# Aceinna/gnss-ins-sim

Measured on AMD Instinct MI355X. Metric: Monte-Carlo IMU samples integrated/sec, higher is better.
Workload: dtype f64

## Files before the change

### gnss-ins-sim_amd/csrc/ginsim_api.hip

```cpp
#include <hip/hip_runtime.h>
#include <chrono>

#include <cmath>
#include <cstdarg>
#include <cstdio>
#include <cstring>
#include <string>
#include <vector>

#include "ginsim.h"
#include "ginsim_oallan.h"
#include "allan.hpp"
#include "oallan.hpp"
#include "comm.hpp"
#include "launch.hpp"
#include "placed.hpp"

namespace ginsim {

static thread_local std::string g_err;

void set_error(const char* fmt, ...) {
    char buf[512];
    va_list ap;
    va_start(ap, fmt);
    vsnprintf(buf, sizeof(buf), fmt, ap);
    va_end(ap);
    g_err = buf;
}

}

using namespace ginsim;

struct ginsim_ctx {
    int device;
    hipStream_t stream;
    hipEvent_t ev0, ev1;
    std::vector<hipEvent_t> pool;
    void* ws[4] = {nullptr, nullptr, nullptr, nullptr};
    size_t ws_bytes[4] = {0, 0, 0, 0};
    double* allan_host = nullptr;
    size_t allan_host_doubles = 0;
    int max_grid_y = 65535;
    ginsim::Comm* comm = nullptr;
    double* comm_recv = nullptr;
    ginsim_stats* comm_host = nullptr;
    hipEvent_t comm_ev[8] = {};
    bool comm_pending[8] = {};
    ginsim_stats* stat_slots = nullptr;
    hipEvent_t stat_ev[8] = {};
    bool stat_pending[8] = {};
    unsigned long long* selftest = nullptr;
};

static hipError_t scratch(ginsim_ctx* c, int slot, size_t bytes, void** out) {
    if (c->ws_bytes[slot] < bytes) {
        if (c->ws[slot]) {
            hipError_t e = hipStreamSynchronize(c->stream);
            if (e != hipSuccess) return e;
            e = hipFree(c->ws[slot]);
            if (e != hipSuccess) return e;
            c->ws[slot] = nullptr;
            c->ws_bytes[slot] = 0;
        }
        const size_t want = bytes + bytes / 4 + 4096;
        hipError_t e = hipMalloc(&c->ws[slot], want);
        if (e != hipSuccess) return e;
        c->ws_bytes[slot] = want;
    }
    *out = c->ws[slot];
    return hipSuccess;
}

#define HIP_TRY(expr)                                                                         \
    do {                                                                                      \
        hipError_t e_ = (expr);                                                               \
        if (e_ != hipSuccess) {                                                               \
            set_error("%s failed: %s (%s:%d)", #expr, hipGetErrorString(e_), __FILE__, __LINE__); \
            if (e_ == hipErrorOutOfMemory) { (void)hipGetLastError(); return GINSIM_ERR_NOMEM; } \
            return GINSIM_ERR_HIP;                                                            \
        }                                                                                     \
    } while (0)

#define REQUIRE(cond, ...)            \
    do {                              \
        if (!(cond)) {                \
            set_error(__VA_ARGS__);   \
            return GINSIM_ERR_ARG;    \
        }                             \
    } while (0)

struct DevBuf {
    void* p = nullptr;
    ~DevBuf() { if (p) (void)hipFree(p); }
    hipError_t alloc(size_t bytes) { return hipMalloc(&p, bytes ? bytes : 8); }
    template <class T> T* as() const { return reinterpret_cast<T*>(p); }
};

template <class Launch>
static int gather_run(const char* who, ginsim_ctx* c, const void* series, int32_t ncomp, int64_t n, int64_t runs, const int64_t* run_ids,
                      int32_t nsel, double* host_out, Launch launch) {
    REQUIRE(c && series && run_ids && host_out, "%s: NULL argument", who);
    REQUIRE(ncomp >= 1 && n >= 1 && runs >= 1 && nsel >= 1, "%s: bad sizes", who);
    for (int i = 0; i < nsel; ++i)
        REQUIRE(run_ids[i] >= 0 && run_ids[i] < runs, "%s: run id %lld out of range", who, (long long)run_ids[i]);
    HIP_TRY(hipSetDevice(c->device));
    DevBuf ids, out;
    const size_t out_bytes = sizeof(double) * (size_t)nsel * n * ncomp;
    HIP_TRY(ids.alloc(sizeof(int64_t) * nsel));
    HIP_TRY(out.alloc(out_bytes));
    HIP_TRY(hipMemcpyAsync(ids.p, run_ids, sizeof(int64_t) * nsel, hipMemcpyHostToDevice, c->stream));
    HIP_TRY(launch(ids.as<int64_t>(), out.as<double>()));
    HIP_TRY(hipMemcpyAsync(host_out, out.p, out_bytes, hipMemcpyDeviceToHost, c->stream));
    HIP_TRY(hipStreamSynchronize(c->stream));
    return GINSIM_OK;
}

template <class Launch>
static int traj_run(ginsim_ctx* c, TrajView v, size_t body, double* host_out, size_t out_bytes, Launch launch) {
    HIP_TRY(hipSetDevice(c->device));
    void* ws = nullptr;
    HIP_TRY(scratch(c, 2, body + sizeof(int64_t) * (size_t)v.m, &ws));
    if (v.samples) {
        int64_t* d_samples = reinterpret_cast<int64_t*>(reinterpret_cast<char*>(ws) + body);
        HIP_TRY(hipMemcpyAsync(d_samples, v.samples, sizeof(int64_t) * (size_t)v.m, hipMemcpyHostToDevice, c->stream));
        v.samples = d_samples;
    }
    HIP_TRY(launch(v, ws));
    if (out_bytes) HIP_TRY(hipMemcpyAsync(host_out, ws, out_bytes, hipMemcpyDeviceToHost, c->stream));
    HIP_TRY(hipStreamSynchronize(c->stream));
    return GINSIM_OK;
}
// ... 125 lines not shown
    int64_t mmax = 0;
    allan_factors(n, fs, mult, &mmax);
    if (mult.empty()) return GINSIM_OK;
    REQUIRE((int)mult.size() <= kOallanMaxFactors && n < ((int64_t)1 << 31), "oallan: series too long");
    const char* e = getenv("GINSIM_OALLAN_TILE");
    const bool tiles = !(e && e[0] == '0' && e[1] == 0);
    const int64_t C = oallan_tile_payload(), H = oallan_tile_halo(), W = oallan_stream_item();
    F.count = (int32_t)mult.size();
    int64_t records = 0;
    for (int i = 0; i < F.count; ++i) {
        const int64_t m = mult[i], terms = n - 2 * m + 1;
        const bool tile = tiles && 2 * m <= H && i == P.tile && P.tile < kOallanTileFactors;
        if (tile) ++P.tile;
        const int64_t per = tile ? C : W;
        F.m[i] = (int32_t)m;
        F.nparts[i] = (int32_t)((terms + per - 1) / per);
        F.offset[i] = (int32_t)records;
        records += F.nparts[i];
    }
    F.records = (int32_t)records;
    const auto pad = [](size_t b) { return (b + 255) & ~(size_t)255; };
    P.b_records = pad(sizeof(double) * (size_t)records * (size_t)nseries);
    if (F.count > P.tile) {
        P.theta_stride = (n + 2) & ~(int64_t)1;
        P.b_theta = pad(sizeof(double) * (size_t)P.theta_stride * (size_t)nseries);
        P.b_sums = pad(sizeof(double) * (size_t)(n / oallan_scan_chunk() + 1) * (size_t)nseries);
    }
    return GINSIM_OK;
}

extern "C" {

int ginsim_abi_version(void) { return GINSIM_ABI_VERSION; }

const char* ginsim_last_error(void) { return g_err.c_str(); }

int ginsim_device_count(int* count) {
    REQUIRE(count, "device_count: NULL output");
    int n = 0;
    const hipError_t e = hipGetDeviceCount(&n);
    if (e != hipSuccess) {
        *count = 0;
        set_error("hipGetDeviceCount: %s", hipGetErrorString(e));
        return GINSIM_ERR_NODEV;
    }
    *count = n;
    return GINSIM_OK;
}

int ginsim_create(int device, ginsim_ctx** out) {
    REQUIRE(out, "create: NULL output");
    *out = nullptr;
    int n = 0;
    if (hipGetDeviceCount(&n) != hipSuccess || n < 1) {
        set_error("no HIP device visible (the engine has no CPU fallback)");
        return GINSIM_ERR_NODEV;
    }
    REQUIRE(device >= 0 && device < n, "create: device %d out of range [0,%d)", device, n);
    HIP_TRY(hipSetDevice(device));
    ginsim_ctx* c = new ginsim_ctx();
    c->device = device;
    HIP_TRY(hipStreamCreateWithFlags(&c->stream, hipStreamNonBlocking));
    HIP_TRY(hipEventCreate(&c->ev0));
    HIP_TRY(hipEventCreate(&c->ev1));
    HIP_TRY(hipDeviceGetAttribute(&c->max_grid_y, hipDeviceAttributeMaxGridDimY, device));
    ginsim::placed_context_created(device);
    *out = c;
    return GINSIM_OK;
}

int ginsim_destroy(ginsim_ctx* c) {
    if (!c) return GINSIM_OK;
    (void)hipSetDevice(c->device);
    (void)hipStreamSynchronize(c->stream);
    (void)hipEventDestroy(c->ev0);
    (void)hipEventDestroy(c->ev1);
    for (hipEvent_t e : c->pool)
        if (e) (void)hipEventDestroy(e);
    for (void* w : c->ws)
        if (w) (void)hipFree(w);
    for (hipEvent_t e : c->stat_ev)
        if (e) (void)hipEventDestroy(e);
    if (c->stat_slots) (void)hipHostFree(c->stat_slots);
    if (c->allan_host) (void)hipHostFree(c->allan_host);
    if (c->selftest) (void)hipFree(c->selftest);
    if (c->comm) ginsim::comm_destroy(c->comm);
    if (c->comm_recv) (void)hipFree(c->comm_recv);
    if (c->comm_host) (void)hipHostFree(c->comm_host);
    for (hipEvent_t e : c->comm_ev)
        if (e) (void)hipEventDestroy(e);
    ginsim::vib_psd_drop_plans(c->stream);
    (void)hipStreamDestroy(c->stream);
    ginsim::placed_free_owner(c->device, c);
    ginsim::placed_context_destroyed(c->device);
    delete c;
    return GINSIM_OK;
}

int ginsim_device_name(ginsim_ctx* c, char* buf, size_t cap) {
    REQUIRE(c && buf && cap > 0, "device_name: bad arguments");
    hipDeviceProp_t prop;
    HIP_TRY(hipGetDeviceProperties(&prop, c->device));
    snprintf(buf, cap, "%s (%s, %d CUs)", prop.name, prop.gcnArchName, prop.multiProcessorCount);
    return GINSIM_OK;
}

int ginsim_malloc(ginsim_ctx* c, size_t bytes, void** dptr) {
    REQUIRE(c && dptr, "malloc: bad arguments");
    HIP_TRY(hipSetDevice(c->device));
    HIP_TRY(hipMalloc(dptr, bytes ? bytes : 8));
    return GINSIM_OK;
}

int ginsim_placed_configure(ginsim_ctx* c, const ginsim_placed_options* o) {
    REQUIRE(c && o, "placed_configure: bad arguments");
    return ginsim::placed_configure(c->device, *o);
}

int ginsim_placed_reserve(ginsim_ctx* c, size_t bytes) {
    REQUIRE(c, "placed_reserve: NULL context");
    return ginsim::placed_reserve(c->device, c->stream, bytes);
}

int ginsim_malloc_placed(ginsim_ctx* c, size_t bytes, void** dptr) {
    REQUIRE(c && dptr, "malloc_placed: bad arguments");
    return ginsim::placed_malloc(c->device, c->stream, bytes, c, dptr);
}

int ginsim_placed_release(ginsim_ctx* c) {
    REQUIRE(c, "placed_release: NULL context");
    HIP_TRY(hipSetDevice(c->device));
    HIP_TRY(hipStreamSynchronize(c->stream));
    return ginsim::placed_release(c->device, false);
}

int ginsim_placed_info_get(ginsim_ctx* c, ginsim_placed_info* out) {
    REQUIRE(c && out, "placed_info_get: bad arguments");
    ginsim::placed_info(c->device, out);
    return GINSIM_OK;
}

int ginsim_mem_info(ginsim_ctx* c, size_t* free_bytes, size_t* total_bytes) {
    REQUIRE(c && free_bytes && total_bytes, "mem_info: bad arguments");
    HIP_TRY(hipSetDevice(c->device));
    HIP_TRY(hipMemGetInfo(free_bytes, total_bytes));
    return GINSIM_OK;
}

int ginsim_host_alloc(ginsim_ctx* c, size_t bytes, void** hptr) {
    REQUIRE(c && hptr, "host_alloc: bad arguments");
    HIP_TRY(hipSetDevice(c->device));
    HIP_TRY(hipHostMalloc(hptr, bytes ? bytes : 8, hipHostMallocDefault));
    return GINSIM_OK;
}

int ginsim_host_free(ginsim_ctx* c, void* hptr) {
    if (!hptr) return GINSIM_OK;
    if (c) {
        HIP_TRY(hipSetDevice(c->device));
        HIP_TRY(hipStreamSynchronize(c->stream));
    }
    HIP_TRY(hipHostFree(hptr));
    return GINSIM_OK;
}

int ginsim_free(ginsim_ctx* c, void* dptr) {
// ... 442 lines not shown
int ginsim_loose_kernel_name(const ginsim_mc_params* mc, const ginsim_loose_params* p, char* buf, size_t cap) {
    REQUIRE(buf && cap > 0, "loose_kernel_name: bad arguments");
    return loose_entry(LOOSE_PLAIN, nullptr, LooseLaunch{mc, p, nullptr, nullptr, nullptr, nullptr, buf, cap});
}

int ginsim_loose_run(ginsim_ctx* c, const ginsim_mc_params* mc, const ginsim_loose_params* p) {
    REQUIRE(c, "loose_run: NULL argument");
    return loose_entry(LOOSE_PLAIN, c, LooseLaunch{mc, p});
}

int ginsim_loose_cons_kernel_name(const ginsim_mc_params* mc, const ginsim_loose_params* p, const ginsim_loose_cons_params* cons,
                                  char* buf, size_t cap) {
    REQUIRE(buf && cap > 0, "loose_cons_kernel_name: bad arguments");
    return loose_entry(LOOSE_CONS, nullptr, LooseLaunch{mc, p, cons, nullptr, nullptr, nullptr, buf, cap});
}

int ginsim_loose_cons_run(ginsim_ctx* c, const ginsim_mc_params* mc, const ginsim_loose_params* p, const ginsim_loose_cons_params* cons) {
    REQUIRE(c, "loose_cons_run: NULL argument");
    return loose_entry(LOOSE_CONS, c, LooseLaunch{mc, p, cons});
}

int ginsim_loose_mag_kernel_name(const ginsim_mc_params* mc, const ginsim_loose_params* p, const ginsim_loose_mag_params* mag,
                                 char* buf, size_t cap) {
    REQUIRE(buf && cap > 0, "loose_mag_kernel_name: bad arguments");
    return loose_entry(LOOSE_MAG, nullptr, LooseLaunch{mc, p, nullptr, mag, nullptr, nullptr, buf, cap});
}

int ginsim_loose_mag_run(ginsim_ctx* c, const ginsim_mc_params* mc, const ginsim_loose_params* p, const ginsim_loose_mag_params* mag) {
    REQUIRE(c, "loose_mag_run: NULL argument");
    return loose_entry(LOOSE_MAG, c, LooseLaunch{mc, p, nullptr, mag});
}

int ginsim_loose_scale_kernel_name(const ginsim_mc_params* mc, const ginsim_loose_params* p, const ginsim_loose_scale_params* scale,
                                   char* buf, size_t cap) {
    REQUIRE(buf && cap > 0, "loose_scale_kernel_name: bad arguments");
    return loose_entry(LOOSE_SCALE, nullptr, LooseLaunch{mc, p, nullptr, nullptr, scale, nullptr, buf, cap});
}

int ginsim_loose_scale_run(ginsim_ctx* c, const ginsim_mc_params* mc, const ginsim_loose_params* p, const ginsim_loose_scale_params* scale) {
    REQUIRE(c, "loose_scale_run: NULL argument");
    return loose_entry(LOOSE_SCALE, c, LooseLaunch{mc, p, nullptr, nullptr, scale});
}

int ginsim_loose_still_kernel_name(const ginsim_mc_params* mc, const ginsim_loose_params* p, const ginsim_loose_still_params* still,
                                   char* buf, size_t cap) {
    REQUIRE(buf && cap > 0, "loose_still_kernel_name: bad arguments");
    return loose_entry(LOOSE_STILL, nullptr, LooseLaunch{mc, p, nullptr, nullptr, nullptr, still, buf, cap});
}

int ginsim_loose_still_run(ginsim_ctx* c, const ginsim_mc_params* mc, const ginsim_loose_params* p, const ginsim_loose_still_params* still) {
    REQUIRE(c, "loose_still_run: NULL argument");
    return loose_entry(LOOSE_STILL, c, LooseLaunch{mc, p, nullptr, nullptr, nullptr, still});
}

int ginsim_aux_sensors(ginsim_ctx* c, const ginsim_aux_params* p) {
    REQUIRE(c && p, "aux_sensors: NULL argument");
    REQUIRE(p->runs >= 1 && p->n >= 0 && p->m >= 0, "aux_sensors: bad sizes");
    REQUIRE(!p->out_gps || p->ref_gps, "aux_sensors: ref_gps missing");
    REQUIRE(!p->out_mag || p->ref_mag, "aux_sensors: ref_mag missing");
    REQUIRE(p->n <= 0xFFFFFFFFll && p->m <= 0xFFFFFFFFll, "aux_sensors: sample index exceeds the RNG counter");
    REQUIRE((double)p->n * (double)p->runs < 5.0e11 && (double)p->m * (double)p->runs < 5.0e11, "aux_sensors: too many elements");
    HIP_TRY(hipSetDevice(c->device));
    HIP_TRY(launch_aux(*p, c->stream));
    return GINSIM_OK;
}

int ginsim_magcal_run(ginsim_ctx* c, const ginsim_magcal_params* p) {
    REQUIRE(c && p, "magcal_run: NULL argument");
    REQUIRE(p->runs >= 1, "magcal_run: runs=%lld must be >= 1", (long long)p->runs);
    REQUIRE(p->n >= 1 && p->n <= 0xFFFFFFFFll, "magcal_run: n must lie in 1 .. the 32-bit sample counter of the RNG");
    REQUIRE(p->runs <= (int64_t)0x7FFFFFFF * 64, "magcal_run: too many runs for one launch");
    REQUIRE(p->in_mag || p->ref_mag, "magcal_run: neither ref_mag (generated form) nor in_mag (given form)");
    REQUIRE(p->out_si && p->out_hi, "magcal_run: out_si / out_hi missing");
    for (int a = 0; a < 3; ++a) {
        const long long s0 = (long long)p->seg[2 * a], s1 = (long long)p->seg[2 * a + 1];
        REQUIRE(s0 >= 0 && s1 <= (long long)p->n, "magcal_run: range %c [%lld, %lld) is outside [0, %lld]", "xyz"[a], s0, s1, (long long)p->n);
        REQUIRE(s0 < s1, "magcal_run: range %c [%lld, %lld) is empty", "xyz"[a], s0, s1);
    }
    HIP_TRY(hipSetDevice(c->device));
    HIP_TRY(launch_magcal(*p, c->stream));
    return GINSIM_OK;
}

int ginsim_end_stats(ginsim_ctx* c, const double* end_err, int64_t runs, ginsim_stats* host_out) {
    REQUIRE(c && end_err && host_out && runs >= 1, "end_stats: bad arguments");
    HIP_TRY(hipSetDevice(c->device));
    void* ws = nullptr;
    HIP_TRY(scratch(c, 0, stats_scratch_bytes(runs), &ws));
    HIP_TRY(launch_end_stats(end_err, runs, ws, c->stream));
    const char* res = reinterpret_cast<char*>(ws) + stats_scratch_bytes(runs) - sizeof(ginsim_stats);
    HIP_TRY(hipMemcpyAsync(host_out, res, sizeof(ginsim_stats), hipMemcpyDeviceToHost, c->stream));
    HIP_TRY(hipStreamSynchronize(c->stream));
    return GINSIM_OK;
}

int ginsim_end_stats_begin(ginsim_ctx* c, const double* end_err, int64_t runs, int32_t slot) {
    REQUIRE(c && end_err && runs >= 1 && slot >= 0 && slot < 8, "end_stats_begin: bad arguments");
    REQUIRE(!c->stat_pending[slot], "end_stats_begin: slot %d is still pending (call ginsim_end_stats_finish first)", slot);
    HIP_TRY(hipSetDevice(c->device));
    if (!c->stat_slots) HIP_TRY(hipHostMalloc(reinterpret_cast<void**>(&c->stat_slots), 8 * sizeof(ginsim_stats), hipHostMallocDefault));
    if (!c->stat_ev[slot]) HIP_TRY(hipEventCreateWithFlags(&c->stat_ev[slot], hipEventDisableTiming));
    void* ws = nullptr;
    HIP_TRY(scratch(c, 0, stats_scratch_bytes(runs), &ws));
    HIP_TRY(launch_end_stats(end_err, runs, ws, c->stream));
    const char* res = reinterpret_cast<char*>(ws) + stats_scratch_bytes(runs) - sizeof(ginsim_stats);
    HIP_TRY(hipMemcpyAsync(&c->stat_slots[slot], res, sizeof(ginsim_stats), hipMemcpyDeviceToHost, c->stream));
    HIP_TRY(hipEventRecord(c->stat_ev[slot], c->stream));
    c->stat_pending[slot] = true;
    return GINSIM_OK;
}

int ginsim_end_stats_finish(ginsim_ctx* c, int32_t slot, ginsim_stats* host_out) {
    REQUIRE(c && host_out && slot >= 0 && slot < 8, "end_stats_finish: bad arguments");
    REQUIRE(c->stat_pending[slot], "end_stats_finish: nothing was begun in slot %d", slot);
    HIP_TRY(hipEventSynchronize(c->stat_ev[slot]));
    *host_out = c->stat_slots[slot];
    c->stat_pending[slot] = false;
    return GINSIM_OK;
}

int ginsim_comm_unique_id(unsigned char* id) {
    REQUIRE(id, "comm_unique_id: NULL output");
    const char* err = comm_unique_id(id);
    if (err) { set_error("comm_unique_id: %s", err); return GINSIM_ERR_HIP; }
    return GINSIM_OK;
}

int ginsim_comm_init(ginsim_ctx* c, int32_t nranks, int32_t rank, const unsigned char* id) {
    REQUIRE(c && id && nranks >= 1 && rank >= 0 && rank < nranks, "comm_init: bad arguments");
    REQUIRE(!c->comm, "comm_init: this context already has a communicator");
    HIP_TRY(hipSetDevice(c->device));
    const size_t bytes = sizeof(ginsim_stats) * 8 * (size_t)nranks;
    hipError_t e = hipMalloc(reinterpret_cast<void**>(&c->comm_recv), bytes);
    if (e == hipSuccess) e = hipHostMalloc(reinterpret_cast<void**>(&c->comm_host), bytes, hipHostMallocDefault);
    const char* err = e == hipSuccess ? comm_create(nranks, rank, id, &c->comm) : nullptr;
    if (e != hipSuccess || err) {
        if (c->comm_recv) { (void)hipFree(c->comm_recv); c->comm_recv = nullptr; }
        if (c->comm_host) { (void)hipHostFree(c->comm_host); c->comm_host = nullptr; }
        c->comm = nullptr;
        if (err) set_error("comm_init: %s", err);
        else set_error("comm_init: %s", hipGetErrorString(e));
        return GINSIM_ERR_HIP;
    }
    return GINSIM_OK;
}

int ginsim_comm_probe(void) {
    const char* err = comm_probe();
    if (err) { set_error("comm_probe: %s", err); return GINSIM_ERR_HIP; }
    return GINSIM_OK;
}

__global__ void first_xcc_kernel(uint32_t* out) {
    if (threadIdx.x == 0) out[0] = __builtin_amdgcn_s_getreg((31 << 11) | 20) & 0xf;
}

int ginsim_stream_first_xcc(ginsim_ctx* c, int32_t* xcc) {
    REQUIRE(c && xcc, "stream_first_xcc: NULL argument");
    HIP_TRY(hipSetDevice(c->device));
    void* ws = nullptr;
    HIP_TRY(scratch(c, 2, 64, &ws));
    hipLaunchKernelGGL(first_xcc_kernel, dim3(1), dim3(64), 0, c->stream, reinterpret_cast<uint32_t*>(ws));
    HIP_TRY(hipGetLastError());
    uint32_t v = 0;
    HIP_TRY(hipMemcpyAsync(&v, ws, sizeof v, hipMemcpyDeviceToHost, c->stream));
    HIP_TRY(hipStreamSynchronize(c->stream));
    *xcc = (int32_t)v;
    return GINSIM_OK;
}

int ginsim_vib_psd_series(ginsim_ctx* c, const double* amp, int64_t period, int64_t runs, uint64_t run_offset, uint64_t seed,
                          int32_t sensor, int32_t halve_per_run, double* out) {
    REQUIRE(c && amp && out, "vib_psd_series: NULL argument");
    REQUIRE(period >= 2 && period <= 16384 && period % 2 == 0, "vib_psd_series: period %lld must be even, 2 .. 16384 (time_series_from_psd.py:36-43)",
            (long long)period);
    REQUIRE(runs >= 1 && runs <= (int64_t)0x7FFFFFFF * 64, "vib_psd_series: runs=%lld out of range", (long long)runs);
    REQUIRE(sensor == 0 || sensor == 1, "vib_psd_series: sensor must be 0 (accelerometer) or 1 (gyroscope)");
    REQUIRE(halve_per_run == 0 || halve_per_run == 1, "vib_psd_series: halve_per_run must be 0 or 1");
    for (int64_t k = 0; k < 3 * (period / 2 + 1); ++k)
        REQUIRE(std::isfinite(amp[k]) && amp[k] >= 0.0, "vib_psd_series: amplitude %lld is negative or not finite", (long long)k);
    HIP_TRY(hipSetDevice(c->device));
    void* ws = nullptr;
    HIP_TRY(scratch(c, 3, vib_psd_scratch_bytes(period, runs), &ws));
    return launch_vib_psd(c->device, c->stream, amp, period, runs, run_offset, seed, sensor, halve_per_run, ws, out);
}

int ginsim_comm_query(ginsim_ctx* c, int32_t* nranks, int32_t* rank, int32_t* device) {
    REQUIRE(c && nranks && rank && device, "comm_query: bad arguments");
    REQUIRE(c->comm, "comm_query: no communicator (ginsim_comm_init)");
    int n = -1, r = -1, d = -1;
    const char* err = comm_query(c->comm, &n, &r, &d);
    if (err) { set_error("comm_query: %s", err); return GINSIM_ERR_HIP; }
    *nranks = n; *rank = r; *device = d;
    return GINSIM_OK;
}

int ginsim_comm_destroy(ginsim_ctx* c) {
    REQUIRE(c, "comm_destroy: NULL context");
    if (!c->comm) return GINSIM_OK;
    HIP_TRY(hipSetDevice(c->device));
    HIP_TRY(hipStreamSynchronize(c->stream));
    comm_destroy(c->comm);
    c->comm = nullptr;
    if (c->comm_recv) { (void)hipFree(c->comm_recv); c->comm_recv = nullptr; }
    if (c->comm_host) { (void)hipHostFree(c->comm_host); c->comm_host = nullptr; }
    for (bool& p : c->comm_pending) p = false;
    return GINSIM_OK;
}

int ginsim_end_stats_all_begin(ginsim_ctx* c, const double* end_err, int64_t runs, int32_t slot) {
    REQUIRE(c && runs >= 0 && (runs == 0 || end_err) && slot >= 0 && slot < 8, "end_stats_all_begin: bad arguments");
    REQUIRE(c->comm && c->comm_recv && c->comm_host, "end_stats_all_begin: no communicator (ginsim_comm_init)");
    REQUIRE(!c->comm_pending[slot], "end_stats_all_begin: slot %d is still pending (call ginsim_end_stats_all_finish first)", slot);
    HIP_TRY(hipSetDevice(c->device));
    if (!c->comm_ev[slot]) HIP_TRY(hipEventCreateWithFlags(&c->comm_ev[slot], hipEventDisableTiming));
    const int nranks = comm_nranks(c->comm);
    void* ws = nullptr;
    const size_t wb = stats_scratch_bytes(runs > 0 ? runs : 1);
    HIP_TRY(scratch(c, 0, wb, &ws));
    double* rec = reinterpret_cast<double*>(reinterpret_cast<char*>(ws) + wb - sizeof(ginsim_stats));
    if (runs > 0) HIP_TRY(launch_end_stats(end_err, runs, ws, c->stream));
    else HIP_TRY(hipMemsetAsync(rec, 0, sizeof(ginsim_stats), c->stream));
    double* recv = c->comm_recv + (size_t)slot * nranks * (sizeof(ginsim_stats) / sizeof(double));
    const char* err = comm_allgather_f64(c->comm, rec, recv, sizeof(ginsim_stats) / sizeof(double), c->stream);
    if (err) { set_error("end_stats_all_begin: %s", err); return GINSIM_ERR_HIP; }
    HIP_TRY(hipMemcpyAsync(c->comm_host + (size_t)slot * nranks, recv, sizeof(ginsim_stats) * nranks, hipMemcpyDeviceToHost, c->stream));
    HIP_TRY(hipEventRecord(c->comm_ev[slot], c->stream));
    c->comm_pending[slot] = true;
    return GINSIM_OK;
}

int ginsim_end_stats_all_finish(ginsim_ctx* c, int32_t slot, ginsim_stats* merged) {
    REQUIRE(c && merged && slot >= 0 && slot < 8, "end_stats_all_finish: bad arguments");
    REQUIRE(c->comm && c->comm_pending[slot], "end_stats_all_finish: nothing was begun in slot %d", slot);
    HIP_TRY(hipEventSynchronize(c->comm_ev[slot]));
    c->comm_pending[slot] = false;
    const int nranks = comm_nranks(c->comm);
    std::vector<ginsim_stats> parts;
    for (int r = 0; r < nranks; ++r) {
        const ginsim_stats& p = c->comm_host[(size_t)slot * nranks + r];
        if (p.count > 0) parts.push_back(p);
    }
    memset(merged, 0, sizeof(*merged));
    if (!parts.empty()) stats_merge_host(parts.data(), (int)parts.size(), merged);
    return GINSIM_OK;
}

static int traj_stats_run(ginsim_ctx* c, const TrajView& v, int64_t first_sample, int32_t pos_ned, double* proc_out, ginsim_stats* end_out) {
    HIP_TRY(hipSetDevice(c->device));
    void* ws = nullptr;
    const size_t bytes = sizeof(double) * 27 * (size_t)v.runs;
    HIP_TRY(scratch(c, 2, bytes, &ws));
    double* rec = reinterpret_cast<double*>(ws);
    HIP_TRY(launch_process_stats(v, proc_out ? first_sample : v.n - 1, pos_ned, proc_out ? 1 : 0, rec, c->stream));
    if (!proc_out) return ginsim_end_stats(c, rec + (size_t)9 * v.runs, v.runs, end_out);
    HIP_TRY(hipMemcpyAsync(proc_out, ws, bytes, hipMemcpyDeviceToHost, c->stream));
    HIP_TRY(hipStreamSynchronize(c->stream));
    return GINSIM_OK;
}

int ginsim_process_stats(ginsim_ctx* c, const double* traj, const double* ref, int64_t n, int64_t runs, int64_t first_sample,
                         int32_t pos_ned, double* host_out) {
    REQUIRE(c && traj && ref && host_out, "process_stats: NULL argument");
    REQUIRE(n >= 1 && runs >= 1 && first_sample >= 0 && first_sample < n, "process_stats: bad sizes");
    return traj_stats_run(c, TrajView{traj, 0, ref, n, runs, nullptr, 0, {nullptr, 0, 0}}, first_sample, pos_ned, host_out, nullptr);
}

int ginsim_end_stats_from_traj(ginsim_ctx* c, const double* traj, const double* ref, int64_t n, int64_t runs, int32_t pos_ned,
                               ginsim_stats* host_out) {
    REQUIRE(c && traj && ref && host_out && n >= 1 && runs >= 1, "end_stats_from_traj: bad arguments");
    return traj_stats_run(c, TrajView{traj, 0, ref, n, runs, nullptr, 0, {nullptr, 0, 0}}, 0, pos_ned, nullptr, host_out);
}

int ginsim_process_stats_f32(ginsim_ctx* c, const float* traj, const double* ref, int64_t n, int64_t runs, int64_t first_sample,
                             int32_t pos_ned, const double* origin, int32_t n_ini, uint64_t ini_first, double* host_out) {
    REQUIRE(c && traj && ref && origin && host_out, "process_stats_f32: NULL argument");
    REQUIRE(n >= 1 && runs >= 1 && first_sample >= 0 && first_sample < n && n_ini >= 1, "process_stats_f32: bad sizes");
    return traj_stats_run(c, TrajView{traj, 1, ref, n, runs, nullptr, 0, {origin, n_ini, ini_first}}, first_sample, pos_ned, host_out, nullptr);
}

int ginsim_end_stats_from_traj_f32(ginsim_ctx* c, const float* traj, const double* ref, int64_t n, int64_t runs, int32_t pos_ned,
                                   const double* origin, int32_t n_ini, uint64_t ini_first, ginsim_stats* host_out) {
    REQUIRE(c && traj && ref && origin && host_out && n >= 1 && runs >= 1 && n_ini >= 1, "end_stats_from_traj_f32: bad arguments");
    return traj_stats_run(c, TrajView{traj, 1, ref, n, runs, nullptr, 0, {origin, n_ini, ini_first}}, 0, pos_ned, nullptr, host_out);
}

static int check_curve_args(const char* who, const void* c, const TrajView& v, const void* host_out) {
    const int64_t n = v.n, m = v.m;
    REQUIRE(c && v.traj && v.ref && host_out, "%s: NULL argument", who);
    REQUIRE(n >= 1 && v.runs >= 1, "%s: n=%lld runs=%lld must be >= 1", who, (long long)n, (long long)v.runs);
    REQUIRE(m >= 1, "%s: m=%lld samples (at least one is needed)", who, (long long)m);
    REQUIRE(v.samples || m == n, "%s: samples == NULL means every sample, so m must be n (m=%lld, n=%lld)", who, (long long)m, (long long)n);
    REQUIRE(m <= 0x7FFFFFFFll, "%s: too many samples for one call", who);
    if (v.samples)
        for (int64_t i = 0; i < m; ++i)
            REQUIRE(v.samples[i] >= 0 && v.samples[i] < n, "%s: sample %lld (entry %lld) is outside [0, %lld)", who, (long long)v.samples[i],
                    (long long)i, (long long)n);
    return GINSIM_OK;
}

static int check_which(const char* who, int32_t which) {
    REQUIRE(which == 0 || which == 1, "%s: which=%d is neither 0 (position) nor 1 (velocity)", who, (int)which);
    return GINSIM_OK;
}

// ... 451 lines not shown
```

### gnss-ins-sim_amd/csrc/launch.hpp

```cpp
#pragma once
#include <hip/hip_runtime.h>
#include <stdint.h>
#include <stdlib.h>
#include "ginsim.h"

namespace ginsim {

void set_error(const char* fmt, ...);

hipError_t launch_mc(const ginsim_mc_params& p, hipStream_t stream, char* name, size_t cap, double* proc_about);
int mc_variant(const ginsim_mc_params& p);

hipError_t launch_mc_f32(const ginsim_mc_params& p, float* truth32, hipStream_t stream, char* name, size_t cap);
size_t mc_f32_truth_bytes(const ginsim_mc_params& p);
int mc_variant_f32(const ginsim_mc_params& p);

bool series_path_applies(const ginsim_mc_params& p);
int series_pass_b(const ginsim_mc_params& p);
int64_t series_chunks(const ginsim_mc_params& p, int32_t* L_out);
hipError_t launch_series(const ginsim_mc_params& p, double* carry, hipStream_t stream);

hipError_t launch_incl(const ginsim_mc_params& p, const ginsim_incl_params& b, hipStream_t stream, char* name, size_t cap);
int incl_variant(const ginsim_mc_params& p);

struct LooseLaunch {
    const ginsim_mc_params* mc;
    const ginsim_loose_params* b;
    const ginsim_loose_cons_params* cons;
    const ginsim_loose_mag_params* mag;
    const ginsim_loose_scale_params* scale;
    const ginsim_loose_still_params* still;
    char* name; size_t cap;
    const int64_t* stamp;
    const int32_t* visible;
    const int64_t* samples;
    hipStream_t stream;
};

hipError_t launch_loose_plain(const LooseLaunch& L);
hipError_t launch_loose_aided(const LooseLaunch& L);
hipError_t launch_loose_cons(const LooseLaunch& L);
hipError_t launch_loose_mag(const LooseLaunch& L);
hipError_t launch_loose_scale(const LooseLaunch& L);
hipError_t launch_loose_still(const LooseLaunch& L);
int loose_variant(const ginsim_mc_params& p);

hipError_t launch_aux(const ginsim_aux_params& p, hipStream_t s);

hipError_t launch_magcal(const ginsim_magcal_params& p, hipStream_t s);

size_t vib_psd_scratch_bytes(int64_t period, int64_t runs);
int launch_vib_psd(int device, hipStream_t stream, const double* amp, int64_t period, int64_t runs, uint64_t run_offset, uint64_t seed,
                   int sensor, int halve, void* scratch, double* out);
void vib_psd_drop_plans(hipStream_t stream);

hipError_t launch_rng_probe(uint64_t seed, uint64_t run, uint32_t stream, int64_t count, double* z0, double* z1,
                            uint32_t* words, hipStream_t stream_h);
hipError_t launch_normal_transform(const uint32_t* words, int64_t count, double* z0, double* z1, hipStream_t s);

hipError_t launch_aos_to_soa(const double* src, double* dst, int64_t R, int64_t n, int C, hipStream_t s);
hipError_t launch_runs_to_series(const double* in, double* out, int C, int64_t n, int64_t R, hipStream_t s);
hipError_t launch_gather_runs(const double* series, int C, int64_t n, int64_t runs, const int64_t* ids, int nsel,
                              double* out, hipStream_t s);
hipError_t launch_gather_series(const double* series, int C, int64_t n, const int64_t* ids, int nsel, double* out, hipStream_t s);
hipError_t launch_gather_runs_f32(const float* series, int C, int64_t n, int64_t runs, const int64_t* ids, int nsel,
                                  double* out, hipStream_t s);

hipError_t launch_pattern_fill(void* p, uint64_t words, uint32_t tag, hipStream_t s);
hipError_t launch_pattern_check(const void* p, uint64_t words, uint32_t tag, unsigned long long* out, hipStream_t s);
hipError_t launch_digest(const void* p, uint64_t words, unsigned long long* out, hipStream_t s);

struct ProcOrigin {
    const double* table;
    int64_t n_ini;
    uint64_t ini_first;
};

struct TrajView {
    const void* traj;
    int f32;
    const double* ref;
    int64_t n, runs;
    const int64_t* samples;
    int64_t m;
    ProcOrigin org;
};

size_t stats_scratch_bytes(int64_t runs);
int stats_blocks(int64_t runs);
hipError_t launch_end_stats(const double* end_err, int64_t runs, void* scratch, hipStream_t s);
void stats_merge_host(const ginsim_stats* parts, int nparts, ginsim_stats* out);
hipError_t launch_process_stats(const TrajView& v, int64_t j0, int pos_ned, int run_major, double* out, hipStream_t s);

size_t error_curve_scratch_bytes(const TrajView& v);
hipError_t launch_error_curve(const TrajView& v, int pos_ned, void* scratch, hipStream_t s);
void curve_merge_host(const double* parts, int nparts, int64_t m, double* out);

hipError_t launch_radial_keys(const TrajView& v, int which, int pos_ned, double* keys, int64_t row_stride, int64_t col0, hipStream_t s);
hipError_t launch_quantile_rows(const double* keys, int64_t rows, int64_t len, int64_t row_stride, const double* probs, int q,
                                double* out, double* count, hipStream_t s);

size_t error_cov_scratch_bytes(const TrajView& v);
hipError_t launch_error_cov(const TrajView& v, int which, int pos_ned, void* scratch, hipStream_t s);
void cov_merge_host(const double* parts, int nparts, int64_t m, double* out);

inline int split_policy() {
    static const int v = [] { const char* e = getenv("GINSIM_SPLIT"); return e ? atoi(e) : -1; }();
    return v;
}

inline bool any_vibration(const ginsim_mc_params& p) { return p.vib_accel.type != GINSIM_VIB_NONE || p.vib_gyro.type != GINSIM_VIB_NONE; }
inline bool any_psd_vibration(const ginsim_mc_params& p) { return p.vib_accel.type == GINSIM_VIB_PSD || p.vib_gyro.type == GINSIM_VIB_PSD; }

inline bool any_white_drift(const ginsim_mc_params& p) {
    bool f = false;
    for (int k = 0; k < 3; ++k)
        f = f || p.accel.white_drift[k] || p.gyro.white_drift[k] || p.accel.bias[k] != 0.0 || p.gyro.bias[k] != 0.0;
    return f;
}

}
```

### gnss-ins-sim_amd/csrc/stats.hip

```cpp
#include <hip/hip_runtime.h>
#include "ginsim.h"
#include "fastmath.hpp"
#include "ins_math.hpp"
#include "traj_error.hpp"

namespace ginsim {

constexpr int kStatBlock = 256;

__device__ __forceinline__ double shift_of(const double* x) {
    const double k = x[0];
    return __builtin_isfinite(k) ? k : 0.0;
}

__global__ void __launch_bounds__(kStatBlock) stats_partial_kernel(const double* __restrict__ e, int64_t runs,
                                                                   Mom* __restrict__ partial) {
    const int comp = blockIdx.y;
    const double* x = e + (int64_t)comp * runs;
    const double k = shift_of(x);
    Mom m{0.0, 0.0, 0.0, 0.0};
    for (int64_t r = (int64_t)blockIdx.x * kStatBlock + threadIdx.x; r < runs; r += (int64_t)gridDim.x * kStatBlock) {
        const double v = x[r] - k;
        m.n += 1.0;
        if (__builtin_isfinite(v) && __builtin_isfinite(m.mean)) {
            const double d = v - m.mean;
            m.mean += d / m.n;
            m.m2 += d * (v - m.mean);
        } else {
            m.mean += v;
            m.m2 = __builtin_nan("");
        }
        m.mx = nan_max(fabs(x[r]), m.mx);
    }
#pragma unroll
    for (int mask = 32; mask >= 1; mask >>= 1) m = merge(m, shfl_xor(m, mask));
    __shared__ Mom wave_part[kStatBlock / 64];
    if ((threadIdx.x & 63) == 0) wave_part[threadIdx.x >> 6] = m;
    __syncthreads();
    if (threadIdx.x == 0) {
        Mom t = wave_part[0];
        for (int w = 1; w < kStatBlock / 64; ++w) t = merge(t, wave_part[w]);
        partial[comp * gridDim.x + blockIdx.x] = t;
    }
}

__global__ void stats_final_kernel(const Mom* __restrict__ partial, int blocks, const double* __restrict__ e, int64_t runs,
                                   ginsim_stats* __restrict__ out) {
    const int c = blockIdx.x;
    Mom t{0.0, 0.0, 0.0, 0.0};
    for (int b = threadIdx.x; b < blocks; b += 64) t = merge(t, partial[c * blocks + b]);
#pragma unroll
    for (int mask = 32; mask >= 1; mask >>= 1) t = merge(t, shfl_xor(t, mask));
    if (threadIdx.x == 0) {
        if (c == 0) out->count = t.n;
        out->mean[c] = shift_of(e + (int64_t)c * runs) + t.mean;
        out->m2[c] = t.m2;
        out->maxabs[c] = t.mx;
    }
}

constexpr int kSeg = 4;

template <typename T>
__global__ void __launch_bounds__(64 * kSeg) process_stats_kernel(const T* __restrict__ traj, const double* __restrict__ ref,
                                                                 int64_t n, int64_t runs, int64_t j0, int pos_ned,
                                                                 int run_major, double* __restrict__ out, const ProcOrigin org) {
    __shared__ Mom part[kSeg][9][64];
    const int lane = threadIdx.x & 63, seg = threadIdx.x >> 6;
    const int64_t r = (int64_t)blockIdx.x * 64 + lane;
    const bool active = r < runs;
    const int64_t plane = n * runs;
    const uniform_ref truth = (uniform_ref)(uintptr_t)ref;
    const int64_t len = n - j0, per = (len + kSeg - 1) / kSeg;
    const int64_t jb = j0 + seg * per, je = (jb + per < n) ? jb + per : n;
    double mean[9], m2[9], mx[9];
#pragma unroll
    for (int c = 0; c < 9; ++c) { mean[c] = 0.0; m2[c] = 0.0; mx[c] = 0.0; }
    double cnt = 0.0;
    double o3[3] = {0.0, 0.0, 0.0};
    if (org.table && active) run_origin(org, r, o3);
    auto error = [&](int64_t j, double (&e)[9]) {
        double x[9], t[9];
#pragma unroll
        for (int c = 0; c < 9; ++c) { x[c] = (double)traj[c * plane + j * runs + r]; t[c] = truth[9 * j + c]; }
        x[3] += o3[0]; x[4] += o3[1]; x[5] += o3[2];
        sample_error(x, t, pos_ned, e);
    };
    if (active) {
        for (int64_t j = jb; j < je; ++j) {
            double e[9];
            error(j, e);
            cnt += 1.0;
            const double icnt = rcp_nr(cnt);
#pragma unroll
            for (int c = 0; c < 9; ++c) {
                const double d = e[c] - mean[c];
                mean[c] = __builtin_fma(d, icnt, mean[c]);
                m2[c] = __builtin_fma(d, e[c] - mean[c], m2[c]);
                mx[c] = nan_max(fabs(e[c]), mx[c]);
            }
        }
        bool bad = false;
#pragma unroll
        for (int c = 0; c < 9; ++c) bad |= !__builtin_isfinite(mx[c]);
        if (bad) {
            double sum[9];
#pragma unroll
            for (int c = 0; c < 9; ++c) sum[c] = 0.0;
            for (int64_t j = jb; j < je; ++j) {
                double e[9];
                error(j, e);
#pragma unroll
                for (int c = 0; c < 9; ++c) sum[c] += e[c];
            }
#pragma unroll
            for (int c = 0; c < 9; ++c)
                if (!__builtin_isfinite(mx[c])) { mean[c] = sum[c] / cnt; m2[c] = __builtin_nan(""); }
        }
    }
#pragma unroll
    for (int c = 0; c < 9; ++c) part[seg][c][lane] = Mom{cnt, mean[c], m2[c], mx[c]};
    __syncthreads();
    if (seg == 0 && active) {
#pragma unroll
        for (int c = 0; c < 9; ++c) {
            Mom t = part[0][c][lane];
#pragma unroll
            for (int k = 1; k < kSeg; ++k) t = merge(t, part[k][c][lane]);
            const double sd = t.n > 0.0 ? sqrt(t.m2 / t.n) : 0.0;
            if (run_major) {
                out[(r * 3 + 0) * 9 + c] = t.mx;
                out[(r * 3 + 1) * 9 + c] = t.mean;
                out[(r * 3 + 2) * 9 + c] = sd;
            } else {
                out[(0 * 9 + c) * runs + r] = t.mx;
                out[(1 * 9 + c) * runs + r] = t.mean;
                out[(2 * 9 + c) * runs + r] = sd;
            }
        }
    }
}

template <typename T>
static hipError_t launch_proc(const TrajView& v, int64_t j0, int pos_ned, int run_major, double* out, hipStream_t s) {
    hipLaunchKernelGGL((process_stats_kernel<T>), dim3((unsigned)((v.runs + 63) / 64)), dim3(64 * kSeg), 0, s,
                       static_cast<const T*>(v.traj), v.ref, v.n, v.runs, j0, pos_ned, run_major, out, v.org);
    return hipGetLastError();
}

hipError_t launch_process_stats(const TrajView& v, int64_t j0, int pos_ned, int run_major, double* out, hipStream_t s) {
    return v.f32 ? launch_proc<float>(v, j0, pos_ned, run_major, out, s) : launch_proc<double>(v, j0, pos_ned, run_major, out, s);
}

int stats_blocks(int64_t runs) {
    int64_t b = (runs + kStatBlock - 1) / kStatBlock;
    return (int)(b < 1 ? 1 : (b > 256 ? 256 : b));
}

size_t stats_scratch_bytes(int64_t runs) { return sizeof(Mom) * 9 * (size_t)stats_blocks(runs) + sizeof(ginsim_stats); }

hipError_t launch_end_stats(const double* end_err, int64_t runs, void* scratch, hipStream_t s) {
    const int blocks = stats_blocks(runs);
    Mom* partial = reinterpret_cast<Mom*>(scratch);
    ginsim_stats* out = reinterpret_cast<ginsim_stats*>(partial + 9 * blocks);
    hipLaunchKernelGGL(stats_partial_kernel, dim3(blocks, 9), dim3(kStatBlock), 0, s, end_err, runs, partial);
    hipLaunchKernelGGL(stats_final_kernel, dim3(9), dim3(64), 0, s, partial, blocks, end_err, runs, out);
    return hipGetLastError();
}

void stats_merge_host(const ginsim_stats* parts, int nparts, ginsim_stats* out) {
    for (int c = 0; c < 9; ++c) {
        Mom t{0.0, 0.0, 0.0, 0.0};
        for (int k = 0; k < nparts; ++k)
            t = merge(t, Mom{parts[k].count, parts[k].mean[c], parts[k].m2[c], parts[k].maxabs[c]});
        out->count = t.n;
        out->mean[c] = t.mean;
        out->m2[c] = t.m2;
        out->maxabs[c] = t.mx;
    }
}

}
```

Baseline: 53.01 billion.

## Fuse end-stats partial and final reductions into one kernel with last-block tickets

Replaces the two-kernel end-of-run statistics reduction with a single kernel. Each block publishes its partial moments, and hierarchical atomic tickets let the last block per component fold them. The result is written straight into mapped pinned host memory, which removes the second launch and the device-to-host memcpy. The old path stays behind an environment variable. The trade-off is correctness reliance on atomic ordering, ticket reset logic, and system-scope writes to host memory.

Result: no change. 52.96 billion (-0.1%).

```diff
diff --git a/gnss-ins-sim_amd/csrc/ginsim_api.hip b/gnss-ins-sim_amd/csrc/ginsim_api.hip
--- a/gnss-ins-sim_amd/csrc/ginsim_api.hip
+++ b/gnss-ins-sim_amd/csrc/ginsim_api.hip
@@ -4,6 +4,7 @@
 #include <cmath>
 #include <cstdarg>
 #include <cstdio>
+#include <cstdlib>
 #include <cstring>
 #include <string>
 #include <vector>
@@ -49,6 +50,8 @@
     hipEvent_t comm_ev[8] = {};
     bool comm_pending[8] = {};
     ginsim_stats* stat_slots = nullptr;
+    ginsim_stats* stat_slots_dev = nullptr;
+    unsigned* stat_tickets = nullptr;
     hipEvent_t stat_ev[8] = {};
     bool stat_pending[8] = {};
     unsigned long long* selftest = nullptr;
@@ -340,6 +343,7 @@
     for (hipEvent_t e : c->stat_ev)
         if (e) (void)hipEventDestroy(e);
     if (c->stat_slots) (void)hipHostFree(c->stat_slots);
+    if (c->stat_tickets) (void)hipFree(c->stat_tickets);
     if (c->allan_host) (void)hipHostFree(c->allan_host);
     if (c->selftest) (void)hipFree(c->selftest);
     if (c->comm) ginsim::comm_destroy(c->comm);
@@ -948,15 +952,49 @@
     return GINSIM_OK;
 }
 
+static bool end_stats_two_launches() {
+    const char* env = getenv("GINSIM_END_STATS_LAUNCHES");
+    return env && atoi(env) == 2;
+}
+
+static int end_stats_setup(ginsim_ctx* c) {
+    if (!c->stat_slots) {
+        HIP_TRY(hipHostMalloc(reinterpret_cast<void**>(&c->stat_slots), 9 * sizeof(ginsim_stats), hipHostMallocDefault));
+        const hipError_t e = hipHostGetDevicePointer(reinterpret_cast<void**>(&c->stat_slots_dev), c->stat_slots, 0);
+        if (e != hipSuccess) { (void)hipHostFree(c->stat_slots); c->stat_slots = nullptr; }
+        HIP_TRY(e);
+    }
+    if (!c->stat_tickets) {
+        unsigned* t = nullptr;
+        HIP_TRY(hipMalloc(reinterpret_cast<void**>(&t), stats_ticket_bytes()));
+        const hipError_t e = hipMemsetAsync(t, 0, stats_ticket_bytes(), c->stream);
+        if (e != hipSuccess) (void)hipFree(t);
+        HIP_TRY(e);
+        c->stat_tickets = t;
+    }
+    return GINSIM_OK;
+}
+
+static const char* two_launch_record(void* ws, int64_t runs) {
+    return reinterpret_cast<char*>(ws) + stats_scratch_bytes(runs) - sizeof(ginsim_stats);
+}
+
 int ginsim_end_stats(ginsim_ctx* c, const double* end_err, int64_t runs, ginsim_stats* host_out) {
     REQUIRE(c && end_err && host_out && runs >= 1, "end_stats: bad arguments");
     HIP_TRY(hipSetDevice(c->device));
     void* ws = nullptr;
     HIP_TRY(scratch(c, 0, stats_scratch_bytes(runs), &ws));
-    HIP_TRY(launch_end_stats(end_err, runs, ws, c->stream));
-    const char* res = reinterpret_cast<char*>(ws) + stats_scratch_bytes(runs) - sizeof(ginsim_stats);
-    HIP_TRY(hipMemcpyAsync(host_out, res, sizeof(ginsim_stats), hipMemcpyDeviceToHost, c->stream));
-    HIP_TRY(hipStreamSynchronize(c->stream));
+    if (end_stats_two_launches()) {
+        HIP_TRY(launch_end_stats_two(end_err, runs, ws, c->stream));
+        HIP_TRY(hipMemcpyAsync(host_out, two_launch_record(ws, runs), sizeof(ginsim_stats), hipMemcpyDeviceToHost, c->stream));
+        HIP_TRY(hipStreamSynchronize(c->stream));
+        return GINSIM_OK;
+    }
+    const int rc = end_stats_setup(c);
+    if (rc != GINSIM_OK) return rc;
+    HIP_TRY(launch_end_stats(end_err, runs, ws, c->stat_tickets, c->stat_slots_dev + 8, c->stream));
+    HIP_TRY(hipStreamSynchronize(c->stream));
+    *host_out = c->stat_slots[8];
     return GINSIM_OK;
 }
 
@@ -964,13 +1002,17 @@
     REQUIRE(c && end_err && runs >= 1 && slot >= 0 && slot < 8, "end_stats_begin: bad arguments");
     REQUIRE(!c->stat_pending[slot], "end_stats_begin: slot %d is still pending (call ginsim_end_stats_finish first)", slot);
     HIP_TRY(hipSetDevice(c->device));
-    if (!c->stat_slots) HIP_TRY(hipHostMalloc(reinterpret_cast<void**>(&c->stat_slots), 8 * sizeof(ginsim_stats), hipHostMallocDefault));
+    const int rc = end_stats_setup(c);
+    if (rc != GINSIM_OK) return rc;
     if (!c->stat_ev[slot]) HIP_TRY(hipEventCreateWithFlags(&c->stat_ev[slot], hipEventDisableTiming));
     void* ws = nullptr;
     HIP_TRY(scratch(c, 0, stats_scratch_bytes(runs), &ws));
-    HIP_TRY(launch_end_stats(end_err, runs, ws, c->stream));
-    const char* res = reinterpret_cast<char*>(ws) + stats_scratch_bytes(runs) - sizeof(ginsim_stats);
-    HIP_TRY(hipMemcpyAsync(&c->stat_slots[slot], res, sizeof(ginsim_stats), hipMemcpyDeviceToHost, c->stream));
+    if (end_stats_two_launches()) {
+        HIP_TRY(launch_end_stats_two(end_err, runs, ws, c->stream));
+        HIP_TRY(hipMemcpyAsync(&c->stat_slots[slot], two_launch_record(ws, runs), sizeof(ginsim_stats), hipMemcpyDeviceToHost, c->stream));
+    } else {
+        HIP_TRY(launch_end_stats(end_err, runs, ws, c->stat_tickets, c->stat_slots_dev + slot, c->stream));
+    }
     HIP_TRY(hipEventRecord(c->stat_ev[slot], c->stream));
     c->stat_pending[slot] = true;
     return GINSIM_OK;
@@ -1085,8 +1127,15 @@
     const size_t wb = stats_scratch_bytes(runs > 0 ? runs : 1);
     HIP_TRY(scratch(c, 0, wb, &ws));
     double* rec = reinterpret_cast<double*>(reinterpret_cast<char*>(ws) + wb - sizeof(ginsim_stats));
-    if (runs > 0) HIP_TRY(launch_end_stats(end_err, runs, ws, c->stream));
-    else HIP_TRY(hipMemsetAsync(rec, 0, sizeof(ginsim_stats), c->stream));
+    if (runs > 0 && end_stats_two_launches()) {
+        HIP_TRY(launch_end_stats_two(end_err, runs, ws, c->stream));
+    } else if (runs > 0) {
+        const int rc = end_stats_setup(c);
+        if (rc != GINSIM_OK) return rc;
+        HIP_TRY(launch_end_stats(end_err, runs, ws, c->stat_tickets, reinterpret_cast<ginsim_stats*>(rec), c->stream));
+    } else {
+        HIP_TRY(hipMemsetAsync(rec, 0, sizeof(ginsim_stats), c->stream));
+    }
     double* recv = c->comm_recv + (size_t)slot * nranks * (sizeof(ginsim_stats) / sizeof(double));
     const char* err = comm_allgather_f64(c->comm, rec, recv, sizeof(ginsim_stats) / sizeof(double), c->stream);
     if (err) { set_error("end_stats_all_begin: %s", err); return GINSIM_ERR_HIP; }
diff --git a/gnss-ins-sim_amd/csrc/launch.hpp b/gnss-ins-sim_amd/csrc/launch.hpp
--- a/gnss-ins-sim_amd/csrc/launch.hpp
+++ b/gnss-ins-sim_amd/csrc/launch.hpp
@@ -88,7 +88,9 @@
 
 size_t stats_scratch_bytes(int64_t runs);
 int stats_blocks(int64_t runs);
-hipError_t launch_end_stats(const double* end_err, int64_t runs, void* scratch, hipStream_t s);
+size_t stats_ticket_bytes();
+hipError_t launch_end_stats(const double* end_err, int64_t runs, void* scratch, unsigned* ticket, ginsim_stats* out, hipStream_t s);
+hipError_t launch_end_stats_two(const double* end_err, int64_t runs, void* scratch, hipStream_t s);
 void stats_merge_host(const ginsim_stats* parts, int nparts, ginsim_stats* out);
 hipError_t launch_process_stats(const TrajView& v, int64_t j0, int pos_ned, int run_major, double* out, hipStream_t s);
 
diff --git a/gnss-ins-sim_amd/csrc/stats.hip b/gnss-ins-sim_amd/csrc/stats.hip
--- a/gnss-ins-sim_amd/csrc/stats.hip
+++ b/gnss-ins-sim_amd/csrc/stats.hip
@@ -13,10 +13,7 @@
     return __builtin_isfinite(k) ? k : 0.0;
 }
 
-__global__ void __launch_bounds__(kStatBlock) stats_partial_kernel(const double* __restrict__ e, int64_t runs,
-                                                                   Mom* __restrict__ partial) {
-    const int comp = blockIdx.y;
-    const double* x = e + (int64_t)comp * runs;
+__device__ __forceinline__ Mom block_moments(const double* __restrict__ x, int64_t runs) {
     const double k = shift_of(x);
     Mom m{0.0, 0.0, 0.0, 0.0};
     for (int64_t r = (int64_t)blockIdx.x * kStatBlock + threadIdx.x; r < runs; r += (int64_t)gridDim.x * kStatBlock) {
@@ -38,24 +35,81 @@
     if ((threadIdx.x & 63) == 0) wave_part[threadIdx.x >> 6] = m;
     __syncthreads();
     if (threadIdx.x == 0) {
-        Mom t = wave_part[0];
-        for (int w = 1; w < kStatBlock / 64; ++w) t = merge(t, wave_part[w]);
-        partial[comp * gridDim.x + blockIdx.x] = t;
-    }
+        m = wave_part[0];
+        for (int w = 1; w < kStatBlock / 64; ++w) m = merge(m, wave_part[w]);
+    }
+    return m;
+}
+
+__device__ __forceinline__ Mom load_agent(const Mom* p) {
+    return Mom{__hip_atomic_load(&p->n, __ATOMIC_RELAXED, __HIP_MEMORY_SCOPE_AGENT), __hip_atomic_load(&p->mean, __ATOMIC_RELAXED, __HIP_MEMORY_SCOPE_AGENT),
+               __hip_atomic_load(&p->m2, __ATOMIC_RELAXED, __HIP_MEMORY_SCOPE_AGENT), __hip_atomic_load(&p->mx, __ATOMIC_RELAXED, __HIP_MEMORY_SCOPE_AGENT)};
+}
+
+template <bool kAgent>
+__device__ __forceinline__ Mom fold_partials(const Mom* part, int blocks, int lane) {
+    Mom t{0.0, 0.0, 0.0, 0.0};
+    for (int b = lane; b < blocks; b += 64) t = merge(t, kAgent ? load_agent(part + b) : part[b]);
+#pragma unroll
+    for (int mask = 32; mask >= 1; mask >>= 1) t = merge(t, shfl_xor(t, mask));
+    return t;
+}
+
+__global__ void __launch_bounds__(kStatBlock) stats_partial_kernel(const double* __restrict__ e, int64_t runs,
+                                                                   Mom* __restrict__ partial) {
+    const int comp = blockIdx.y;
+    const Mom t = block_moments(e + (int64_t)comp * runs, runs);
+    if (threadIdx.x == 0) partial[comp * gridDim.x + blockIdx.x] = t;
 }
 
 __global__ void stats_final_kernel(const Mom* __restrict__ partial, int blocks, const double* __restrict__ e, int64_t runs,
                                    ginsim_stats* __restrict__ out) {
     const int c = blockIdx.x;
-    Mom t{0.0, 0.0, 0.0, 0.0};
-    for (int b = threadIdx.x; b < blocks; b += 64) t = merge(t, partial[c * blocks + b]);
-#pragma unroll
-    for (int mask = 32; mask >= 1; mask >>= 1) t = merge(t, shfl_xor(t, mask));
+    const Mom t = fold_partials<false>(partial + c * blocks, blocks, threadIdx.x);
     if (threadIdx.x == 0) {
         if (c == 0) out->count = t.n;
         out->mean[c] = shift_of(e + (int64_t)c * runs) + t.mean;
         out->m2[c] = t.m2;
         out->maxabs[c] = t.mx;
+    }
+}
+
+constexpr unsigned kTicketGroup = 8;
+constexpr unsigned kTicketGroups = 256 / kTicketGroup;
+constexpr unsigned kTicketWords = 16 + 9 * kTicketGroups;
+
+__global__ void __launch_bounds__(kStatBlock) stats_kernel(const double* __restrict__ e, int64_t runs, Mom* partial,
+                                                           unsigned* ticket, ginsim_stats* out) {
+    const int comp = blockIdx.y;
+    const double* x = e + (int64_t)comp * runs;
+    const Mom m = block_moments(x, runs);
+    if (threadIdx.x >= 64) return;
+    Mom* part = partial + comp * gridDim.x;
+    int last = 0;
+    if (threadIdx.x == 0) {
+        Mom* p = part + blockIdx.x;
+        __hip_atomic_store(&p->n, m.n, __ATOMIC_RELAXED, __HIP_MEMORY_SCOPE_AGENT);
+        __hip_atomic_store(&p->mean, m.mean, __ATOMIC_RELAXED, __HIP_MEMORY_SCOPE_AGENT);
+        __hip_atomic_store(&p->m2, m.m2, __ATOMIC_RELAXED, __HIP_MEMORY_SCOPE_AGENT);
+        __hip_atomic_store(&p->mx, m.mx, __ATOMIC_RELAXED, __HIP_MEMORY_SCOPE_AGENT);
+        asm volatile("s_waitcnt vmcnt(0)" ::: "memory");
+        const unsigned group = blockIdx.x / kTicketGroup, groups = (gridDim.x + kTicketGroup - 1) / kTicketGroup;
+        const unsigned members = group + 1 < groups ? kTicketGroup : gridDim.x - kTicketGroup * (groups - 1);
+        unsigned* gt = ticket + 16 + comp * kTicketGroups + group;
+        if (__hip_atomic_fetch_add(gt, 1u, __ATOMIC_RELAXED, __HIP_MEMORY_SCOPE_AGENT) == members - 1) {
+            __hip_atomic_store(gt, 0u, __ATOMIC_RELAXED, __HIP_MEMORY_SCOPE_AGENT);
+            last = __hip_atomic_fetch_add(&ticket[comp], 1u, __ATOMIC_RELAXED, __HIP_MEMORY_SCOPE_AGENT) == groups - 1;
+        }
+    }
+    if (!__shfl(last, 0, 64)) return;
+    __builtin_amdgcn_fence(__ATOMIC_ACQUIRE, "agent");
+    const Mom t = fold_partials<true>(part, (int)gridDim.x, threadIdx.x);
+    if (threadIdx.x == 0) {
+        if (comp == 0) __hip_atomic_store(&out->count, t.n, __ATOMIC_RELAXED, __HIP_MEMORY_SCOPE_SYSTEM);
+        __hip_atomic_store(&out->mean[comp], shift_of(x) + t.mean, __ATOMIC_RELAXED, __HIP_MEMORY_SCOPE_SYSTEM);
+        __hip_atomic_store(&out->m2[comp], t.m2, __ATOMIC_RELAXED, __HIP_MEMORY_SCOPE_SYSTEM);
+        __hip_atomic_store(&out->maxabs[comp], t.mx, __ATOMIC_RELAXED, __HIP_MEMORY_SCOPE_SYSTEM);
+        __hip_atomic_store(&ticket[comp], 0u, __ATOMIC_RELAXED, __HIP_MEMORY_SCOPE_AGENT);
     }
 }
 
@@ -157,9 +211,17 @@
     return (int)(b < 1 ? 1 : (b > 256 ? 256 : b));
 }
 
+size_t stats_ticket_bytes() { return sizeof(unsigned) * kTicketWords; }
+
 size_t stats_scratch_bytes(int64_t runs) { return sizeof(Mom) * 9 * (size_t)stats_blocks(runs) + sizeof(ginsim_stats); }
 
-hipError_t launch_end_stats(const double* end_err, int64_t runs, void* scratch, hipStream_t s) {
+hipError_t launch_end_stats(const double* end_err, int64_t runs, void* scratch, unsigned* ticket, ginsim_stats* out, hipStream_t s) {
+    const int blocks = stats_blocks(runs);
+    hipLaunchKernelGGL(stats_kernel, dim3(blocks, 9), dim3(kStatBlock), 0, s, end_err, runs, reinterpret_cast<Mom*>(scratch), ticket, out);
+    return hipGetLastError();
+}
+
+hipError_t launch_end_stats_two(const double* end_err, int64_t runs, void* scratch, hipStream_t s) {
     const int blocks = stats_blocks(runs);
     Mom* partial = reinterpret_cast<Mom*>(scratch);
     ginsim_stats* out = reinterpret_cast<ginsim_stats*>(partial + 9 * blocks);
```
